# microsoft/Spartan

Hardware: AMD Instinct MI355X
Metric: R1CS constraints/sec in SNARK::prove (synthetic 2^20); bit-exact proof (higher is better)
Workload: dtype u64x4 (F_q Montgomery / F_p 2^255-19 limbs)

## Files before the change

### spartan_amd/csrc/spark.hip

```cpp
#include "internal.hpp"

__global__ void __launch_bounds__(256) k_from_index(const uint32_t* __restrict__ ix, size_t n, Fq* __restrict__ dst) { SP_FG_PRIO();
  for (size_t i = (size_t)blockIdx.x * blockDim.x + threadIdx.x; i < n; i += (size_t)gridDim.x * blockDim.x) st_fq(dst + i, fq_from_u64(ix[i]));
}
__global__ void __launch_bounds__(256) k_gather(const Fq* __restrict__ mem, const uint32_t* __restrict__ addr, size_t n, Fq* __restrict__ dst) { SP_FG_PRIO();
  for (size_t i = (size_t)blockIdx.x * blockDim.x + threadIdx.x; i < n; i += (size_t)gridDim.x * blockDim.x) st_fq(dst + i, ld_fq(mem + addr[i]));
}
__global__ void __launch_bounds__(256) k_hash_layer(const Fq* __restrict__ addr, const Fq* __restrict__ val, const Fq* __restrict__ ts, int ts_inc,
                                                    size_t n, Fq r_hash, Fq r_hash_sqr, Fq r_multiset, Fq* __restrict__ dst) { SP_FG_PRIO();
  for (size_t i = (size_t)blockIdx.x * blockDim.x + threadIdx.x; i < n; i += (size_t)gridDim.x * blockDim.x) {
    Fq a = addr ? ld_fq(addr + i) : fq_from_u64((uint64_t)i);
    Fq t = ts ? ld_fq(ts + i) : fq_zero();
    if (ts_inc) t = fq_add(t, fq_one());
    Fq h = fq_add(fq_add(fq_mul(t, r_hash_sqr), fq_mul(ld_fq(val + i), r_hash)), a);
    st_fq(dst + i, fq_sub(h, r_multiset));
  }
}
template <bool PAIR>
__global__ void __launch_bounds__(256) k_hash_layer_first(const Fq* __restrict__ addr, const Fq* __restrict__ val, const Fq* __restrict__ ts, int ts_inc,
                                                          size_t n, Fq r_hash, Fq r_hash_sqr, Fq r_multiset, Fq* __restrict__ dst_a, Fq* __restrict__ dst_b) { SP_FG_PRIO();
  const size_t half = n / 2;
  for (size_t i = (size_t)blockIdx.x * blockDim.x + threadIdx.x; i < half; i += (size_t)gridDim.x * blockDim.x) {
    Fq h[2];
#pragma unroll
    for (int k = 0; k < 2; k++) {
      const size_t j = i + (size_t)k * half;
      Fq a = addr ? ld_fq(addr + j) : fq_from_u64((uint64_t)j);
      Fq t = ts ? ld_fq(ts + j) : fq_zero();
      if (ts_inc) t = fq_add(t, fq_one());
      h[k] = fq_sub(fq_add(fq_add(fq_mul(t, r_hash_sqr), fq_mul(ld_fq(val + j), r_hash)), a), r_multiset);
      st_fq(dst_a + j, h[k]);
    }
    st_fq(dst_a + n + i, fq_mul(h[0], h[1]));
    if (PAIR) {
      Fq w0 = fq_add(h[0], r_hash_sqr), w1 = fq_add(h[1], r_hash_sqr);
      st_fq(dst_b + i, w0);
      st_fq(dst_b + half + i, w1);
      st_fq(dst_b + n + i, fq_mul(w0, w1));
    }
  }
}
__global__ void __launch_bounds__(256) k_prod_layer(const Fq* __restrict__ in, size_t half, Fq* __restrict__ out) { SP_FG_PRIO();
  for (size_t i = (size_t)blockIdx.x * blockDim.x + threadIdx.x; i < half; i += (size_t)gridDim.x * blockDim.x)
    st_fq(out + i, fq_mul(ld_fq(in + i), ld_fq(in + half + i)));
}

struct Stores16 {
  Fq* p[16];
};
__global__ void __launch_bounds__(256) k_prod_layer_many(Stores16 st, size_t off, size_t half, size_t noff) { SP_FG_PRIO();
  const Fq* in = st.p[blockIdx.y] + off;
  Fq* out = st.p[blockIdx.y] + noff;
  for (size_t i = (size_t)blockIdx.x * blockDim.x + threadIdx.x; i < half; i += (size_t)gridDim.x * blockDim.x)
    st_fq(out + i, fq_mul(ld_fq(in + i), ld_fq(in + half + i)));
}

__global__ void __launch_bounds__(256) k_prod_layer2_many(Stores16 st, size_t off, size_t len) { SP_FG_PRIO();
  const size_t q = len / 4, off1 = off + len, off2 = off1 + len / 2;
  Fq* base = st.p[blockIdx.y];
  for (size_t i = (size_t)blockIdx.x * blockDim.x + threadIdx.x; i < q; i += (size_t)gridDim.x * blockDim.x) {
    const Fq x0 = ld_fq(base + off + i), x1 = ld_fq(base + off + q + i), x2 = ld_fq(base + off + 2 * q + i), x3 = ld_fq(base + off + 3 * q + i);
    const Fq lo = fq_mul(x0, x2), hi = fq_mul(x1, x3);
    st_fq(base + off1 + i, lo);
    st_fq(base + off1 + q + i, hi);
    st_fq(base + off2 + i, fq_mul(lo, hi));
  }
}
__global__ void __launch_bounds__(256) k_prod_layer_tail(Stores16 st, size_t off, size_t len) { SP_FG_PRIO();
  __shared__ Fq cur[1024];
  Fq* base = st.p[blockIdx.x];
  size_t half = len / 2, noff = off + len;
  for (size_t i = threadIdx.x; i < half; i += 256) {
    Fq v = fq_mul(ld_fq(base + off + i), ld_fq(base + off + half + i));
    cur[i] = v;
    st_fq(base + noff + i, v);
  }
  __syncthreads();
  len = half;
  while (len > 2) {
    half = len / 2;
    noff += len;
    Fq v[2];
    int n = 0;
    for (size_t i = threadIdx.x; i < half; i += 256) v[n++] = fq_mul(cur[i], cur[half + i]);
    __syncthreads();
    n = 0;
    for (size_t i = threadIdx.x; i < half; i += 256) { cur[i] = v[n]; st_fq(base + noff + i, v[n]); n++; }
    __syncthreads();
    len = half;
  }
}

struct Triple {
  Fq *a, *b, *c;
  Fq* c_out;
};
struct TripleInline { Triple t[24]; };
__device__ __forceinline__ void cubic_point(const Fq& a0, const Fq& a1, const Fq& b0, const Fq& b1, const Fq& c0, const Fq& c1, Fq (&e)[3]) {
  Fq da = fq_sub(a1, a0), db = fq_sub(b1, b0), dc = fq_sub(c1, c0);
  Fq a2 = fq_add(a1, da), b2 = fq_add(b1, db), c2 = fq_add(c1, dc);
  Fq a3 = fq_add(a2, da), b3 = fq_add(b2, db), c3 = fq_add(c2, dc);
  e[0] = fq_add(e[0], fq_mul(fq_mul(a0, b0), c0));
  e[1] = fq_add(e[1], fq_mul(fq_mul(a2, b2), c2));
  e[2] = fq_add(e[2], fq_mul(fq_mul(a3, b3), c3));
}
__global__ void __launch_bounds__(256) k_cubic_eval_batched(const Triple* __restrict__ T, TripleInline IN, size_t half, Fq* __restrict__ partials) { SP_FG_PRIO();
  __shared__ Fq sm[256];
  Triple t = T ? T[blockIdx.y] : IN.t[blockIdx.y];
  Fq e[3] = {fq_zero(), fq_zero(), fq_zero()};
  for (size_t i = (size_t)blockIdx.x * blockDim.x + threadIdx.x; i < half; i += (size_t)gridDim.x * blockDim.x)
    cubic_point(ld_fq(t.a + i), ld_fq(t.a + half + i), ld_fq(t.b + i), ld_fq(t.b + half + i), ld_fq(t.c + i), ld_fq(t.c + half + i), e);
  block_sum_fq<3>(e, sm);
  if (threadIdx.x == 0) {
    Fq* p = partials + ((size_t)blockIdx.y * gridDim.x + blockIdx.x) * 3;
    st_fq(p, e[0]); st_fq(p + 1, e[1]); st_fq(p + 2, e[2]);
  }
}
__global__ void __launch_bounds__(256) k_cubic_bind_eval_batched(const Triple* __restrict__ T, TripleInline IN, size_t quarter, Fq r, Fq* __restrict__ partials) { SP_FG_PRIO();
  __shared__ Fq sm[256];
  Triple t = T ? T[blockIdx.y] : IN.t[blockIdx.y];
  Fq e[3] = {fq_zero(), fq_zero(), fq_zero()};
  for (size_t i = (size_t)blockIdx.x * blockDim.x + threadIdx.x; i < quarter; i += (size_t)gridDim.x * blockDim.x) {
    Fq lo[3], hi[3];
    Fq* ptr[3] = {t.a, t.b, t.c};
#pragma unroll
    for (int k = 0; k < 3; k++) {
      Fq x0 = ld_fq(ptr[k] + i), x1 = ld_fq(ptr[k] + quarter + i), x2 = ld_fq(ptr[k] + 2 * quarter + i), x3 = ld_fq(ptr[k] + 3 * quarter + i);
      lo[k] = fq_add(x0, fq_mul(r, fq_sub(x2, x0)));
      hi[k] = fq_add(x1, fq_mul(r, fq_sub(x3, x1)));
      if (k < 2) {
        st_fq(ptr[k] + i, lo[k]);
        st_fq(ptr[k] + quarter + i, hi[k]);
      } else if (t.c_out) {
        st_fq(t.c_out + i, lo[k]);
        st_fq(t.c_out + quarter + i, hi[k]);
      }
    }
    cubic_point(lo[0], hi[0], lo[1], hi[1], lo[2], hi[2], e);
  }
  block_sum_fq<3>(e, sm);
  if (threadIdx.x == 0) {
    Fq* p = partials + ((size_t)blockIdx.y * gridDim.x + blockIdx.x) * 3;
    st_fq(p, e[0]); st_fq(p + 1, e[1]); st_fq(p + 2, e[2]);
  }
}
__device__ __forceinline__ void quad_point_eq(const Fq& a0, const Fq& a1, const Fq& b0, const Fq& b1, const Fq& c, Fq (&e)[4]) {
  Fq a2 = fq_add(a1, fq_sub(a1, a0)), b2 = fq_add(b1, fq_sub(b1, b0));
  e[0] = fq_add(e[0], fq_mul(fq_mul(a0, b0), c));
  e[1] = fq_add(e[1], fq_mul(fq_mul(a2, b2), c));
}
__device__ __forceinline__ void cubic_point4(const Fq& a0, const Fq& a1, const Fq& b0, const Fq& b1, const Fq& c0, const Fq& c1, Fq (&e)[4]) {
  Fq da = fq_sub(a1, a0), db = fq_sub(b1, b0), dc = fq_sub(c1, c0);
  Fq a2 = fq_add(a1, da), b2 = fq_add(b1, db), c2 = fq_add(c1, dc);
  Fq a3 = fq_add(a2, da), b3 = fq_add(b2, db), c3 = fq_add(c2, dc);
  e[0] = fq_add(e[0], fq_mul(fq_mul(a0, b0), c0));
  e[1] = fq_add(e[1], fq_mul(fq_mul(a1, b1), c1));
  e[2] = fq_add(e[2], fq_mul(fq_mul(a2, b2), c2));
  e[3] = fq_add(e[3], fq_mul(fq_mul(a3, b3), c3));
}
template <bool GEN>
__global__ void __launch_bounds__(256) k_cubic_eval_batched_eq(TripleInline IN, unsigned inst0, size_t half, Fq* __restrict__ partials) { SP_FG_PRIO();
  __shared__ Fq sm[256];
  const unsigned inst = inst0 + blockIdx.y;
  Triple t = IN.t[inst];
  Fq e[4] = {fq_zero(), fq_zero(), fq_zero(), fq_zero()};
  if (!GEN) {
    for (size_t i = (size_t)blockIdx.x * blockDim.x + threadIdx.x; i < half; i += (size_t)gridDim.x * blockDim.x)
      quad_point_eq(ld_fq(t.a + i), ld_fq(t.a + half + i), ld_fq(t.b + i), ld_fq(t.b + half + i), ld_fq(t.c + i), e);
  } else {
    for (size_t i = (size_t)blockIdx.x * blockDim.x + threadIdx.x; i < half; i += (size_t)gridDim.x * blockDim.x)
      cubic_point4(ld_fq(t.a + i), ld_fq(t.a + half + i), ld_fq(t.b + i), ld_fq(t.b + half + i), ld_fq(t.c + i), ld_fq(t.c + half + i), e);
  }
  if (GEN) block_sum_fq<4>(e, sm);
  else {
    Fq q[2] = {e[0], e[1]};
    block_sum_fq<2>(q, sm);
    e[0] = q[0]; e[1] = q[1];
  }
  if (threadIdx.x == 0) {
    Fq* p = partials + ((size_t)inst * gridDim.x + blockIdx.x) * 4;
    st_fq(p, e[0]); st_fq(p + 1, e[1]); st_fq(p + 2, e[2]); st_fq(p + 3, e[3]);
  }
}
template <bool GEN>
__global__ void __launch_bounds__(256) k_cubic_bind_eval_batched_eq(TripleInline IN, unsigned inst0, size_t quarter, Fq r, Fq* __restrict__ partials) { SP_FG_PRIO();
  __shared__ Fq sm[256];
  const unsigned inst = inst0 + blockIdx.y;
  Triple t = IN.t[inst];
  Fq e[4] = {fq_zero(), fq_zero(), fq_zero(), fq_zero()};
  for (size_t i = (size_t)blockIdx.x * blockDim.x + threadIdx.x; i < quarter; i += (size_t)gridDim.x * blockDim.x) {
    Fq lo[3], hi[3];
    Fq* ptr[3] = {t.a, t.b, t.c};
#pragma unroll
    for (int k = 0; k < 2; k++) {
      Fq x0 = ld_fq(ptr[k] + i), x1 = ld_fq(ptr[k] + quarter + i), x2 = ld_fq(ptr[k] + 2 * quarter + i), x3 = ld_fq(ptr[k] + 3 * quarter + i);
      lo[k] = fq_add(x0, fq_mul(r, fq_sub(x2, x0)));
      hi[k] = fq_add(x1, fq_mul(r, fq_sub(x3, x1)));
      st_fq(ptr[k] + i, lo[k]);
      st_fq(ptr[k] + quarter + i, hi[k]);
    }
    if (!GEN) {
      quad_point_eq(lo[0], hi[0], lo[1], hi[1], ld_fq(t.c + i), e);
    } else {
      Fq x0 = ld_fq(ptr[2] + i), x1 = ld_fq(ptr[2] + quarter + i), x2 = ld_fq(ptr[2] + 2 * quarter + i), x3 = ld_fq(ptr[2] + 3 * quarter + i);
      lo[2] = fq_add(x0, fq_mul(r, fq_sub(x2, x0)));
      hi[2] = fq_add(x1, fq_mul(r, fq_sub(x3, x1)));
      if (t.c_out) {
        st_fq(t.c_out + i, lo[2]);
        st_fq(t.c_out + quarter + i, hi[2]);
      }
      cubic_point4(lo[0], hi[0], lo[1], hi[1], lo[2], hi[2], e);
    }
  }
  if (GEN) block_sum_fq<4>(e, sm);
  else {
    Fq q[2] = {e[0], e[1]};
    block_sum_fq<2>(q, sm);
    e[0] = q[0]; e[1] = q[1];
  }
  if (threadIdx.x == 0) {
    Fq* p = partials + ((size_t)inst * gridDim.x + blockIdx.x) * 4;
    st_fq(p, e[0]); st_fq(p + 1, e[1]); st_fq(p + 2, e[2]); st_fq(p + 3, e[3]);
  }
}
__global__ void __launch_bounds__(256) k_scale_prefix(Fq* __restrict__ t, size_t n, Fq k) { SP_FG_PRIO();
  for (size_t i = (size_t)blockIdx.x * blockDim.x + threadIdx.x; i < n; i += (size_t)gridDim.x * blockDim.x) st_fq(t + i, fq_mul(ld_fq(t + i), k));
}
__global__ void __launch_bounds__(256) k_cubic_bind_eval_tiny(const Triple* __restrict__ T, TripleInline IN, size_t quarter, Fq r, Fq* __restrict__ partials, DoneSig sig) { SP_FG_PRIO();
  __shared__ Fq bound[32][6];
  __shared__ Fq lv[32][3][3];
  __shared__ Fq red[3][32];
  Triple t = T ? T[blockIdx.y] : IN.t[blockIdx.y];
  int li = threadIdx.x >> 3, role = threadIdx.x & 7;
  size_t i = (size_t)blockIdx.x * 32 + li;
  bool live = i < quarter;
  if (role < 6 && live) {
    int k = role >> 1, half = role & 1;
    Fq* ptr = k == 0 ? t.a : (k == 1 ? t.b : t.c);
    Fq x0 = ld_fq(ptr + (size_t)half * quarter + i), x2 = ld_fq(ptr + (size_t)(2 + half) * quarter + i);
    Fq v = fq_add(x0, fq_mul(r, fq_sub(x2, x0)));
    bound[li][role] = v;
    if (k < 2) st_fq(ptr + (size_t)half * quarter + i, v);
    else if (t.c_out) st_fq(t.c_out + (size_t)half * quarter + i, v);
  }
  __syncthreads();
  if (role < 3 && live) {
    const Fq lo = bound[li][2 * role], hi = bound[li][2 * role + 1];
    const Fq d = fq_sub(hi, lo), e2 = fq_add(hi, d), e3 = fq_add(e2, d);
    lv[li][role][0] = lo; lv[li][role][1] = e2; lv[li][role][2] = e3;
  }
  __syncthreads();
  if (role < 3) {
    Fq e = fq_zero();
    if (live) e = fq_mul(fq_mul(lv[li][0][role], lv[li][1][role]), lv[li][2][role]);
    red[role][li] = e;
  }
  __syncthreads();
  for (int s = 16; s > 0; s >>= 1) {
    if (role < 3 && li < s) red[role][li] = fq_add(red[role][li], red[role][li + s]);
    __syncthreads();
  }
  if (threadIdx.x < 3) st_fq(partials + ((size_t)blockIdx.y * gridDim.x + blockIdx.x) * 3 + threadIdx.x, red[threadIdx.x][0]);
  signal_done(sig);
}
__global__ void __launch_bounds__(256) k_cubic_eval_tiny(const Triple* __restrict__ T, TripleInline IN, size_t half, Fq* __restrict__ partials, DoneSig sig) { SP_FG_PRIO();
  __shared__ Fq red[3][64];
  Triple t = T ? T[blockIdx.y] : IN.t[blockIdx.y];
  int li = threadIdx.x >> 2, role = threadIdx.x & 3;
  size_t i = (size_t)blockIdx.x * 64 + li;
  Fq e = fq_zero();
  if (role < 3 && i < half) {
    Fq pt[3];
    const Fq* ptr[3] = {t.a, t.b, t.c};
#pragma unroll
    for (int k = 0; k < 3; k++) {
      Fq x0 = ld_fq(ptr[k] + i), x1 = ld_fq(ptr[k] + half + i);
      Fq x2 = fq_sub(fq_dbl(x1), x0), x3 = fq_sub(fq_add(x2, x1), x0);
#pragma unroll
      for (int w = 0; w < 4; w++) pt[k].l[w] = role == 0 ? x0.l[w] : (role == 1 ? x2.l[w] : x3.l[w]);
    }
    e = fq_mul(fq_mul(pt[0], pt[1]), pt[2]);
  }
  if (role < 3) red[role][li] = e;
  __syncthreads();
  for (int s = 32; s > 0; s >>= 1) {
    if (role < 3 && li < s) red[role][li] = fq_add(red[role][li], red[role][li + s]);
    __syncthreads();
  }
  if (threadIdx.x < 3) st_fq(partials + ((size_t)blockIdx.y * gridDim.x + blockIdx.x) * 3 + threadIdx.x, red[threadIdx.x][0]);
  signal_done(sig);
}

struct Triple2 {
  Fq *a, *b, *c;
  Fq* c_out;
};
__device__ __forceinline__ Fq line_at(const Fq& u, const Fq& v, int t) {
  Fq x2 = fq_sub(fq_dbl(v), u), x3 = fq_sub(fq_add(x2, v), u), r;
#pragma unroll
  for (int w = 0; w < 4; w++) r.l[w] = t == 0 ? u.l[w] : (t == 1 ? x2.l[w] : x3.l[w]);
  return r;
}
struct Bind2Inline {
  Triple2 t[24];
  Fq w[24];
};
__global__ void __launch_bounds__(256) k_cubic_bind2_eval(const Triple2* __restrict__ T, Bind2Inline IN, const Fq* __restrict__ weights, size_t len, int nbind, Fq r0, Fq r1,
                                                          Fq* __restrict__ partials, Fq* __restrict__ dump, DoneSig sig) { SP_FG_PRIO();
  __shared__ Fq first[8][12][2];
  __shared__ Fq bnd[8][12];
  __shared__ Fq red[18][8];
  __shared__ Fq lv[8][3][6][3];
  DoneSig kt = sig; if (blockIdx.x != 0 || blockIdx.y != 0) kt.kt = nullptr;
  SP_KT(kt, 0);
  const Triple2 t = T ? T[blockIdx.y] : IN.t[blockIdx.y];
  const Fq wv = !weights ? fq_zero() : (T ? ld_fq(weights + blockIdx.y) : IN.w[blockIdx.y]);
  const int grp = threadIdx.x >> 5, lane = threadIdx.x & 31;
  const size_t n2 = len >> nbind;
  const size_t np = n2 < 4 ? n2 : 4, ng = n2 / np;
  const size_t g = (size_t)blockIdx.x * 8 + grp;
  const bool live = g < ng;
  Fq* const ptr[3] = {t.a, t.b, t.c};
  if (nbind) {
    if (nbind == 2) {
      if (live && lane < 24) {
        const int k = lane >> 3, p = (lane >> 1) & 3, h = lane & 1;
        if ((size_t)p < np) {
          const size_t y = g + (size_t)p * ng + (size_t)h * (len / 4);
          Fq lo = ld_fq(ptr[k] + y), hi = ld_fq(ptr[k] + y + len / 2);
          SP_KT(kt, 1);
          first[grp][k * 4 + p][h] = fq_add(lo, fq_mul(r0, fq_sub(hi, lo)));
        }
      }
      SP_KT(kt, 2);
      __syncthreads();
    }
    if (live && lane < 12) {
      const int k = lane >> 2, p = lane & 3;
      if ((size_t)p < np) {
        Fq lo, hi;
        if (nbind == 2) { lo = first[grp][lane][0]; hi = first[grp][lane][1]; }
        else { lo = ld_fq(ptr[k] + g + (size_t)p * ng); hi = ld_fq(ptr[k] + g + (size_t)p * ng + len / 2); }
        Fq v = fq_add(lo, fq_mul(nbind == 2 ? r1 : r0, fq_sub(hi, lo)));
        const size_t z = g + (size_t)p * ng;
        if (k < 2) st_fq(ptr[k] + z, v);
        else if (t.c_out) st_fq(t.c_out + z, v);
        if (dump) st_fq(dump + ((size_t)blockIdx.y * 3 + k) * 8 + z, v);
        bnd[grp][k * 4 + (np == 2 && p == 1 ? 2 : p)] = v;
      }
    }
  } else if (live && lane < 12) {
    const int k = lane >> 2, p = lane & 3;
    if ((size_t)p < np) {
      const Fq v = ld_fq(ptr[k] + g + (size_t)p * ng);
      if (dump) st_fq(dump + ((size_t)blockIdx.y * 3 + k) * 8 + g + (size_t)p * ng, v);
      bnd[grp][k * 4 + (np == 2 && p == 1 ? 2 : p)] = v;
    }
  }
  SP_KT(kt, 3);
  __syncthreads();
  if (live && lane < 12 && np >= 2) {
    const int k = lane >> 2, line = lane & 3;
    if (line == 0 || np == 4) {
      const int iu = line == 0 ? 0 : (line == 1 ? 1 : (line == 2 ? 0 : 2)), iv = line == 0 ? 2 : (line == 1 ? 3 : (line == 2 ? 1 : 3));
// ... 176 lines not shown
    size_t half = len / 2, noff = off + len;
    ProfScope ps(c, PF_SPARK, 48.0 * (double)len);
    hipLaunchKernelGGL(k_prod_layer, dim3((unsigned)grid_for(half)), dim3(256), 0, c->stream, (const Fq*)(store->d + off), half, store->d + noff);
    off = noff;
    len = half;
  }
  return hipGetLastError() == hipSuccess ? SP_OK : SP_EHIP;
}

int32_t sp_product_tree_many(sp_ctx* c, sp_table* const* stores, size_t count, size_t n) { return sp_product_tree_many_from(c, stores, count, n, 0); }
int32_t sp_product_tree_many_from(sp_ctx* c, sp_table* const* stores, size_t count, size_t n, size_t layers_done) {
  if (!c || !stores || count == 0 || !is_pow2(n) || n < 2 || layers_done > 1 || (layers_done == 1 && n < 4)) return SP_EINVAL;
  for (size_t k = 0; k < count; k++)
    if (!stores[k] || stores[k]->cap < 2 * n) return SP_EINVAL;
  HIPCHK(hipSetDevice(c->dev));
  for (size_t k0 = 0; k0 < count; k0 += 16) {
    size_t nk = count - k0 < 16 ? count - k0 : 16;
    Stores16 st;
    for (size_t k = 0; k < 16; k++) st.p[k] = k < nk ? stores[k0 + k]->d : nullptr;
    size_t off = 0, len = n;
    if (layers_done == 1) { off = n; len = n / 2; }
    while (len > 2) {
      size_t half = len / 2, noff = off + len;
      ProfScope ps(c, PF_SPARK, 48.0 * (double)len * (double)nk);
      if (len <= 2048) {
        hipLaunchKernelGGL(k_prod_layer_tail, dim3((unsigned)nk), dim3(256), 0, c->stream, st, off, len);
        break;
      }
      const bool two_layers = c->opt.v[OPT_SPARK_PROD_LAYER2] != 0;
      const size_t l2max = (size_t)1 << (c->opt.v[OPT_SPARK_PROD_LAYER2_MAX_LOG2] < 13 ? 13 : c->opt.v[OPT_SPARK_PROD_LAYER2_MAX_LOG2]);
      if (two_layers && len <= l2max && len >= 8192) {
        hipLaunchKernelGGL(k_prod_layer2_many, dim3((unsigned)grid_for(len / 4, 1024), (unsigned)nk), dim3(256), 0, c->stream, st, off, len);
        off = off + len + len / 2;
        len = len / 4;
        continue;
      }
      hipLaunchKernelGGL(k_prod_layer_many, dim3((unsigned)grid_for(half, 1024), (unsigned)nk), dim3(256), 0, c->stream, st, off, half, noff);
      off = noff;
      len = half;
    }
  }
  return hipGetLastError() == hipSuccess ? SP_OK : SP_EHIP;
}

static int32_t batched_setup(sp_ctx* c, sp_table* const* A, sp_table* const* B, sp_table* const* C, size_t ninst, size_t* len_out, bool bind_c, TripleInline* IN,
                             const Triple** Tdev) {
  if (!c || !A || !B || !C || ninst == 0 || ninst > 64) return SP_EINVAL;
  size_t len = A[0] ? A[0]->len : 0;
  std::vector<Triple> T(ninst);
  for (size_t k = 0; k < ninst; k++) {
    if (!A[k] || !B[k] || !C[k] || A[k]->len != len || B[k]->len != len || C[k]->len != len) return SP_EINVAL;
    T[k] = Triple{A[k]->d, B[k]->d, C[k]->d, nullptr};
  }
  if (len < 2 || !is_pow2(len)) return SP_EINVAL;
  if (bind_c) {
    for (size_t k = 0; k < ninst; k++) {
      bool first = true;
      for (size_t m = 0; m < k; m++) first = first && C[m] != C[k];
      if (first) {
        SPCHK(table_ensure_alt(C[k], len / 2));
        T[k].c_out = C[k]->alt;
      }
    }
  }
  const bool inline_args = c->opt.v[OPT_SUMCHECK_INLINE_ARGS] != 0;
  if (inline_args && ninst <= 24) {
    memcpy(IN->t, T.data(), sizeof(Triple) * ninst);
    *Tdev = nullptr;
  } else {
    stage_small(c, 0, T.data(), sizeof(Triple) * ninst);
    *Tdev = (const Triple*)c->hmap;
  }
  *len_out = len;
  return SP_OK;
}
static bool host_sums(size_t nblk, size_t ninst) { return nblk == 1 || 96 * nblk * ninst <= HOST_SUM_BYTES; }
static int32_t batched_finish(sp_ctx* c, Fq* partials, size_t nblk, size_t ninst, uint64_t* out, const DoneSig& sig) {
  if (partials != (Fq*)hres(c)) {
    {
      ProfScope ps(c, PF_REDUCE, 96.0 * (double)(nblk * ninst));
      hipLaunchKernelGGL(k_reduce_partials_batched, dim3((unsigned)ninst), dim3(256), 0, c->stream, (const Fq*)partials, nblk, 3, (Fq*)hres(c), sig);
    }
    SPCHK(sig_wait(c, sig));
    memcpy(out, hres(c), 96 * ninst);
    return hipGetLastError() == hipSuccess ? SP_OK : SP_EHIP;
  }
  SPCHK(sig_wait(c, sig));
  if (hipGetLastError() != hipSuccess) return SP_EHIP;
  const Fq* p = (const Fq*)hres(c);
  Fq* o = (Fq*)out;
  for (size_t i = 0; i < ninst; i++)
    for (int k = 0; k < 3; k++) {
      Fq acc = p[(i * nblk) * 3 + k];
      for (size_t b = 1; b < nblk; b++) acc = fq_add(acc, p[(i * nblk + b) * 3 + k]);
      o[3 * i + k] = acc;
    }
  return SP_OK;
}
int32_t sp_sumcheck_eval_batched(sp_ctx* c, sp_table* const* A, sp_table* const* B, sp_table* const* C, size_t ninst, uint64_t* out) {
  if (!out) return SP_EINVAL;
  size_t len;
  HIPCHK(hipSetDevice(c ? c->dev : 0));
  TripleInline IN;
  const Triple* Tdev = nullptr;
  SPCHK(batched_setup(c, A, B, C, ninst, &len, false, &IN, &Tdev));
  size_t half = len / 2;
  bool tiny = half <= 8192;
  size_t nblk = tiny ? (half + 63) / 64 : grid_for(half, 256);
  SPCHK(ensure(&c->scratch, &c->scratch_cap, 32 * 3 * (nblk + 1) * ninst));
  bool on_host = host_sums(nblk, ninst) && tiny;
  Fq* partials = on_host ? (Fq*)hres(c) : (Fq*)c->scratch;
  DoneSig sig = sig_make(c, on_host ? nblk * ninst : ninst);
  {
    ProfScope ps(c, PF_SC_EVAL, 96.0 * (double)len * (double)ninst, nullptr, 6.0 * (double)half * (double)ninst);
    if (tiny) hipLaunchKernelGGL(k_cubic_eval_tiny, dim3((unsigned)nblk, (unsigned)ninst), dim3(256), 0, c->stream, Tdev, IN, half, partials, on_host ? sig : sig_none());
    else hipLaunchKernelGGL(k_cubic_eval_batched, dim3((unsigned)nblk, (unsigned)ninst), dim3(256), 0, c->stream, Tdev, IN, half, partials);
  }
  return batched_finish(c, partials, nblk, ninst, out, sig);
}
int32_t sp_sumcheck_bind_eval_batched(sp_ctx* c, sp_table* const* A, sp_table* const* B, sp_table* const* C, size_t ninst, const uint64_t r[4],
                                      uint64_t* out) {
  if (!out || !r) return SP_EINVAL;
  size_t len;
  HIPCHK(hipSetDevice(c ? c->dev : 0));
  if (!c) return SP_EINVAL;
  for (size_t k = 0; k < ninst && C; k++)
    if (C[k] && C[k]->len < 4) return SP_EINVAL;
  TripleInline IN;
  const Triple* Tdev = nullptr;
  SPCHK(batched_setup(c, A, B, C, ninst, &len, true, &IN, &Tdev));
  if (len < 4) return SP_EINVAL;
  size_t quarter = len / 4;
  bool tiny = quarter <= 8192;
  size_t nblk = tiny ? (quarter + 31) / 32 : grid_for(quarter, 256);
  SPCHK(ensure(&c->scratch, &c->scratch_cap, 32 * 3 * (nblk + 1) * ninst));
  bool on_host = host_sums(nblk, ninst) && tiny;
  Fq* partials = on_host ? (Fq*)hres(c) : (Fq*)c->scratch;
  DoneSig sig = sig_make(c, on_host ? nblk * ninst : ninst);
  {
    ProfScope ps(c, PF_SC_BIND_EVAL, (96.0 + 32.0) * (double)len * (double)ninst, nullptr, 12.0 * (double)quarter * (double)ninst);
    if (tiny)
      hipLaunchKernelGGL(k_cubic_bind_eval_tiny, dim3((unsigned)nblk, (unsigned)ninst), dim3(256), 0, c->stream, Tdev, IN, quarter,
                         limbs(r), partials, on_host ? sig : sig_none());
    else
      hipLaunchKernelGGL(k_cubic_bind_eval_batched, dim3((unsigned)nblk, (unsigned)ninst), dim3(256), 0, c->stream, Tdev, IN, quarter,
                         limbs(r), partials);
  }
  for (size_t k = 0; k < ninst; k++) { A[k]->len = len / 2; B[k]->len = len / 2; }
  for (size_t k = 0; k < ninst; k++)
    if (C[k]->len == len) table_swap_to_alt(C[k], len / 2);
  return batched_finish(c, partials, nblk, ninst, out, sig);
}

static int32_t batched_finish4(sp_ctx* c, Fq* partials, size_t nblk, size_t ninst, uint64_t* out, const DoneSig& sig) {
  {
    ProfScope ps(c, PF_REDUCE, 128.0 * (double)(nblk * ninst));
    hipLaunchKernelGGL(k_reduce_partials_batched, dim3((unsigned)ninst), dim3(256), 0, c->stream, (const Fq*)partials, nblk, 4, (Fq*)hres(c), sig);
  }
  SPCHK(sig_wait(c, sig));
  memcpy(out, hres(c), 128 * ninst);
  return hipGetLastError() == hipSuccess ? SP_OK : SP_EHIP;
}
static int32_t eq_form_check(sp_table* const* C, size_t ninst, size_t neq, size_t len) {
  if (neq == 0 || neq > ninst || ninst > 24 || 128 * ninst > HOST_SUM_BYTES) return SP_EINVAL;
  for (size_t k = 0; k < neq; k++)
    if (C[k] != C[0]) return SP_EINVAL;
  if (!C[0] || C[0]->len < len) return SP_EINVAL;
  for (size_t k = neq; k < ninst; k++)
    if (!C[k] || C[k]->len != len || C[k] == C[0]) return SP_EINVAL;
  return SP_OK;
}
static int32_t eq_form_setup(sp_ctx* c, sp_table* const* A, sp_table* const* B, sp_table* const* C, size_t ninst, size_t neq, bool bind_c, size_t* len_out,
                             TripleInline* IN) {
  if (!c || !A || !B || !C || ninst == 0) return SP_EINVAL;
  const size_t len = A[0] ? A[0]->len : 0;
  if (len < 65536 || !is_pow2(len)) return SP_EINVAL;
  SPCHK(eq_form_check(C, ninst, neq, len));
  for (size_t k = 0; k < ninst; k++) {
    if (!A[k] || !B[k] || A[k]->len != len || B[k]->len != len) return SP_EINVAL;
    IN->t[k] = Triple{A[k]->d, B[k]->d, C[k]->d, nullptr};
    if (bind_c && k >= neq) {
      bool first = true;
      for (size_t m = neq; m < k; m++) first = first && C[m] != C[k];
      if (first) {
        SPCHK(table_ensure_alt(C[k], len / 2));
        IN->t[k].c_out = C[k]->alt;
      }
    }
  }
  *len_out = len;
  return SP_OK;
}
int32_t sp_sumcheck_eval_batched_eq(sp_ctx* c, sp_table* const* A, sp_table* const* B, sp_table* const* C, size_t ninst, size_t neq, uint64_t* out) {
  if (!c || !out) return SP_EINVAL;
  HIPCHK(hipSetDevice(c->dev));
  size_t len;
  TripleInline IN;
  SPCHK(eq_form_setup(c, A, B, C, ninst, neq, false, &len, &IN));
  const size_t half = len / 2, nblk = grid_for(half, 256);
  SPCHK(ensure(&c->scratch, &c->scratch_cap, 32 * 4 * (nblk + 1) * ninst));
  Fq* partials = (Fq*)c->scratch;
  DoneSig sig = sig_make(c, ninst);
  {
    ProfScope ps(c, PF_SC_EVAL, 32.0 * (double)len * (2.5 * (double)neq + 3.0 * (double)(ninst - neq)), nullptr,
                 (double)half * (4.0 * (double)neq + 8.0 * (double)(ninst - neq)));
    hipLaunchKernelGGL(k_cubic_eval_batched_eq<false>, dim3((unsigned)nblk, (unsigned)neq), dim3(256), 0, c->stream, IN, 0u, half, partials);
    if (ninst > neq)
      hipLaunchKernelGGL(k_cubic_eval_batched_eq<true>, dim3((unsigned)nblk, (unsigned)(ninst - neq)), dim3(256), 0, c->stream, IN, (unsigned)neq, half, partials);
  }
  return batched_finish4(c, partials, nblk, ninst, out, sig);
}
int32_t sp_sumcheck_bind_eval_batched_eq(sp_ctx* c, sp_table* const* A, sp_table* const* B, sp_table* const* C, size_t ninst, size_t neq, const uint64_t r[4],
                                         uint64_t* out) {
  if (!c || !out || !r) return SP_EINVAL;
  HIPCHK(hipSetDevice(c->dev));
  size_t len;
  TripleInline IN;
  SPCHK(eq_form_setup(c, A, B, C, ninst, neq, true, &len, &IN));
  const size_t quarter = len / 4, nblk = grid_for(quarter, 256);
  SPCHK(ensure(&c->scratch, &c->scratch_cap, 32 * 4 * (nblk + 1) * ninst));
  Fq* partials = (Fq*)c->scratch;
  DoneSig sig = sig_make(c, ninst);
  {
    ProfScope ps(c, PF_SC_BIND_EVAL, 32.0 * (double)len * (3.25 * (double)neq + 4.0 * (double)(ninst - neq)), nullptr,
                 (double)quarter * (8.0 * (double)neq + 14.0 * (double)(ninst - neq)));
    hipLaunchKernelGGL(k_cubic_bind_eval_batched_eq<false>, dim3((unsigned)nblk, (unsigned)neq), dim3(256), 0, c->stream, IN, 0u, quarter, limbs(r), partials);
    if (ninst > neq)
      hipLaunchKernelGGL(k_cubic_bind_eval_batched_eq<true>, dim3((unsigned)nblk, (unsigned)(ninst - neq)), dim3(256), 0, c->stream, IN, (unsigned)neq, quarter,
                         limbs(r), partials);
  }
  for (size_t k = 0; k < ninst; k++) { A[k]->len = len / 2; B[k]->len = len / 2; }
  for (size_t k = neq; k < ninst; k++)
    if (C[k]->len == len) table_swap_to_alt(C[k], len / 2);
  return batched_finish4(c, partials, nblk, ninst, out, sig);
}
int32_t sp_table_scale_prefix(sp_ctx* c, sp_table* t, size_t n, const uint64_t k[4]) {
  if (!c || !t || !k || n == 0 || n > t->len) return SP_EINVAL;
  HIPCHK(hipSetDevice(c->dev));
  {
    ProfScope ps(c, PF_MISC, 64.0 * (double)n);
    hipLaunchKernelGGL(k_scale_prefix, dim3((unsigned)grid_for(n)), dim3(256), 0, c->stream, t->d, n, limbs(k));
  }
  t->len = n;
  return hipGetLastError() == hipSuccess ? SP_OK : SP_EHIP;
}

__global__ void __launch_bounds__(256) k_reduce_partials18(const Fq* __restrict__ partials, size_t nblk, Fq* __restrict__ out, DoneSig sig) { SP_FG_PRIO();
  __shared__ Fq sm[8][18];
  const int k = threadIdx.x & 31, sl = threadIdx.x >> 5;
  const Fq* p = partials + (size_t)blockIdx.x * nblk * 18;
  if (k < 18) {
    Fq acc = fq_zero();
    for (size_t b = sl; b < nblk; b += 8) acc = fq_add(acc, ld_fq(p + b * 18 + k));
    sm[sl][k] = acc;
  }
  __syncthreads();
  if (threadIdx.x < 18) {
    Fq acc = sm[0][threadIdx.x];
#pragma unroll
    for (int j = 1; j < 8; j++) acc = fq_add(acc, sm[j][threadIdx.x]);
    st_fq(out + (size_t)blockIdx.x * 18 + threadIdx.x, acc);
  }
  signal_done(sig);
}
constexpr size_t TAIL_OFF = 12288, TAIL_MAX_INST = 21;
struct Bind2Shape {
  size_t n2, nblk;
  bool host, tail;
};
static Bind2Shape bind2_shape(size_t len, int nbind, size_t ninst, bool want_tables) {
  Bind2Shape s;
  s.n2 = len >> nbind;
  const size_t np = s.n2 < 4 ? s.n2 : 4, ng = s.n2 / np;
  s.nblk = (ng + 7) / 8;
  s.host = 32 * 18 * s.nblk * ninst <= HOST_SUM_BYTES;
  s.tail = want_tables && s.n2 >= 2 && s.n2 <= 8 && ninst <= TAIL_MAX_INST && s.host && s.nblk == 1;
  return s;
}
static void bind2_enqueue(sp_ctx* c, const Bind2Inline& IN, bool inl, const Fq* dweights, size_t len, int nbind, const Fq& r0, const Fq& r1, size_t ninst,
                          const Bind2Shape& sh, const DoneSig& sig) {
  const size_t ng = sh.n2 / (sh.n2 < 4 ? sh.n2 : 4);
  Fq* partials = sh.host ? (Fq*)hres(c) : (Fq*)c->scratch;
  Fq* dump = sh.tail ? (Fq*)(hres(c) + TAIL_OFF) : nullptr;
  {
    ProfScope ps(c, nbind ? PF_SC_BIND_EVAL : PF_SC_EVAL, 96.0 * (double)len * (double)ninst, nullptr, (nbind ? 36.0 + 36.0 : 36.0) * (double)ng * (double)ninst);
    hipLaunchKernelGGL(k_cubic_bind2_eval, dim3((unsigned)sh.nblk, (unsigned)ninst), dim3(256), 0, c->stream, inl ? (const Triple2*)nullptr : (const Triple2*)c->hmap, IN, dweights, len,
                       nbind, r0, r1, partials, dump, sh.host ? sig : sig_none());
  }
  if (!sh.host) {
    ProfScope ps(c, PF_REDUCE, 32.0 * 18 * (double)(sh.nblk * ninst));
    hipLaunchKernelGGL(k_reduce_partials18, dim3((unsigned)ninst), dim3(256), 0, c->stream, (const Fq*)partials, sh.nblk, (Fq*)hres(c), sig);
  }
}
static int32_t bind2_launch(sp_ctx* c, sp_table* const* A, sp_table* const* B, sp_table* const* C, size_t ninst, int nbind, const uint64_t* r0, const uint64_t* r1,
                            const uint64_t* weights, uint64_t* out_evals, uint64_t* out_coeffs, uint64_t* out_heads, uint64_t* out_tables = nullptr) {
  if (!c || !A || !B || !C || ninst == 0 || ninst > 64) return SP_EINVAL;
  HIPCHK(hipSetDevice(c->dev));
  size_t len = A[0] ? A[0]->len : 0;
  if (len < ((size_t)1 << nbind) || len < 2 || !is_pow2(len)) return SP_EINVAL;
  const int do_bind = nbind;
  const size_t n2 = len >> nbind;
  if ((n2 >= 2 && !out_evals) || (n2 >= 4 && !out_coeffs) || (n2 == 1 && !out_heads)) return SP_EINVAL;
  for (size_t k = 0; k < ninst; k++)
    if (!A[k] || !B[k] || !C[k] || A[k]->len != len || B[k]->len != len || C[k]->len != len) return SP_EINVAL;
  std::vector<Triple2> T(ninst);
  std::vector<sp_table*> distinctC;
  for (size_t k = 0; k < ninst; k++) {
    T[k] = Triple2{A[k]->d, B[k]->d, C[k]->d, nullptr};
    bool first = true;
    for (size_t m = 0; m < k; m++) first = first && C[m] != C[k];
    if (first) {
      distinctC.push_back(C[k]);
      if (do_bind) {
        SPCHK(table_ensure_alt(C[k], n2));
        T[k].c_out = C[k]->alt;
      }
    }
  }
  const bool inline_args = c->opt.v[OPT_SUMCHECK_INLINE_ARGS] != 0;
  const bool inl = inline_args && ninst <= 24;
  Bind2Inline IN;
  const Fq* dweights = nullptr;
  if (inl) {
    memcpy(IN.t, T.data(), sizeof(Triple2) * ninst);
    if (weights) { memcpy(IN.w, weights, 32 * ninst); dweights = (const Fq*)c->hmap; }
  } else {
    stage_small(c, 0, T.data(), sizeof(Triple2) * ninst);
    dweights = weights ? (const Fq*)stage_small(c, sizeof(Triple2) * 64, weights, 32 * ninst) : nullptr;
  }
  const Bind2Shape sh = bind2_shape(len, nbind, ninst, out_tables != nullptr);
  const Fq z = fq_zero();
  SPCHK(ensure(&c->scratch, &c->scratch_cap, 32 * 18 * (sh.nblk + 1) * ninst));
  const DoneSig sig = sig_make(c, sh.host ? sh.nblk * ninst : ninst);
  bind2_enqueue(c, IN, inl, dweights, len, nbind, r0 ? limbs(r0) : z, r1 ? limbs(r1) : z, ninst, sh, sig);
  if (do_bind) {
    for (size_t k = 0; k < ninst; k++) { A[k]->len = n2; B[k]->len = n2; }
    for (sp_table* t : distinctC) table_swap_to_alt(t, n2);
  }
  SPCHK(sig_wait(c, sig));
  std::vector<Fq> sums(18 * ninst);
  if (!sh.host) {
    memcpy(sums.data(), hres(c), 32 * 18 * ninst);
  } else {
    const Fq* p = (const Fq*)hres(c);
    for (size_t i = 0; i < ninst; i++)
      for (int k = 0; k < 18; k++) {
        Fq acc = p[(i * sh.nblk) * 18 + k];
        for (size_t b = 1; b < sh.nblk; b++) acc = fq_add(acc, p[(i * sh.nblk + b) * 18 + k]);
        sums[18 * i + k] = acc;
      }
  }
  if (hipGetLastError() != hipSuccess) return SP_EHIP;
  if (out_tables) {
    if (sh.tail) {
      const Fq* d = (const Fq*)(hres(c) + TAIL_OFF);
      for (size_t i = 0; i < ninst; i++)
        for (int k = 0; k < 3; k++) memcpy(out_tables + 4 * ((i * 3 + k) * n2), d + (i * 3 + k) * 8, 32 * n2);
    } else {
      out_tables[0] = ~0ULL;
    }
  }
  if (weights) {
    Fq tot[15];
    for (int k = 0; k < 15; k++) {
      Fq acc = sums[k];
      for (size_t i = 1; i < ninst; i++) acc = fq_add(acc, sums[18 * i + k]);
      tot[k] = acc;
    }
    if (n2 >= 2) memcpy(out_evals, tot, 96);
    if (n2 >= 4) memcpy(out_coeffs, tot + 3, 384);
  }
  for (size_t i = 0; i < ninst; i++) {
// ... 92 lines not shown
```

Baseline: 47.21 million.

## Prefetch next grid-stride loads in eq sumcheck kernels and size grids per CU

The batched eq-form sumcheck eval and bind-eval kernels now software-pipeline their grid-stride loops, loading the next iteration's operands into registers before computing on the current ones. The grid for these kernels is now sized from the CU count (about two workgroups per CU spread across instances, with a minimum number of trips per thread) instead of one thread per element. The aim is to hide memory latency and cut the cost of per-block partial reductions. The prefetch raises register pressure on these u64x4 field kernels, which could lower occupancy or cause spills.

```diff
diff --git a/spartan_amd/csrc/spark.hip b/spartan_amd/csrc/spark.hip
--- a/spartan_amd/csrc/spark.hip
+++ b/spartan_amd/csrc/spark.hip
@@ -158,18 +158,41 @@
   e[2] = fq_add(e[2], fq_mul(fq_mul(a2, b2), c2));
   e[3] = fq_add(e[3], fq_mul(fq_mul(a3, b3), c3));
 }
+struct FqPair { Fq lo, hi; };
+struct FqQuad { Fq x0, x1, x2, x3; };
+__device__ __forceinline__ FqPair ld_pair(const Fq* p, size_t half, size_t i) { return FqPair{ld_fq(p + i), ld_fq(p + half + i)}; }
+__device__ __forceinline__ FqQuad ld_quad(const Fq* p, size_t quarter, size_t i) {
+  return FqQuad{ld_fq(p + i), ld_fq(p + quarter + i), ld_fq(p + 2 * quarter + i), ld_fq(p + 3 * quarter + i)};
+}
+__device__ __forceinline__ FqPair bind_quad(const FqQuad& q, const Fq& r) {
+  return FqPair{fq_add(q.x0, fq_mul(r, fq_sub(q.x2, q.x0))), fq_add(q.x1, fq_mul(r, fq_sub(q.x3, q.x1)))};
+}
 template <bool GEN>
 __global__ void __launch_bounds__(256) k_cubic_eval_batched_eq(TripleInline IN, unsigned inst0, size_t half, Fq* __restrict__ partials) { SP_FG_PRIO();
   __shared__ Fq sm[256];
   const unsigned inst = inst0 + blockIdx.y;
   Triple t = IN.t[inst];
   Fq e[4] = {fq_zero(), fq_zero(), fq_zero(), fq_zero()};
-  if (!GEN) {
-    for (size_t i = (size_t)blockIdx.x * blockDim.x + threadIdx.x; i < half; i += (size_t)gridDim.x * blockDim.x)
-      quad_point_eq(ld_fq(t.a + i), ld_fq(t.a + half + i), ld_fq(t.b + i), ld_fq(t.b + half + i), ld_fq(t.c + i), e);
-  } else {
-    for (size_t i = (size_t)blockIdx.x * blockDim.x + threadIdx.x; i < half; i += (size_t)gridDim.x * blockDim.x)
-      cubic_point4(ld_fq(t.a + i), ld_fq(t.a + half + i), ld_fq(t.b + i), ld_fq(t.b + half + i), ld_fq(t.c + i), ld_fq(t.c + half + i), e);
+  const size_t stride = (size_t)gridDim.x * blockDim.x;
+  size_t i = (size_t)blockIdx.x * blockDim.x + threadIdx.x;
+  FqPair na = {fq_zero(), fq_zero()}, nb = na, nc = na;
+  if (i < half) {
+    na = ld_pair(t.a, half, i);
+    nb = ld_pair(t.b, half, i);
+    nc.lo = ld_fq(t.c + i);
+    if (GEN) nc.hi = ld_fq(t.c + half + i);
+  }
+  for (; i < half; i += stride) {
+    const FqPair a = na, b = nb, c = nc;
+    const size_t j = i + stride;
+    if (j < half) {
+      na = ld_pair(t.a, half, j);
+      nb = ld_pair(t.b, half, j);
+      nc.lo = ld_fq(t.c + j);
+      if (GEN) nc.hi = ld_fq(t.c + half + j);
+    }
+    if (!GEN) quad_point_eq(a.lo, a.hi, b.lo, b.hi, c.lo, e);
+    else cubic_point4(a.lo, a.hi, b.lo, b.hi, c.lo, c.hi, e);
   }
   if (GEN) block_sum_fq<4>(e, sm);
   else {
@@ -188,28 +211,48 @@
   const unsigned inst = inst0 + blockIdx.y;
   Triple t = IN.t[inst];
   Fq e[4] = {fq_zero(), fq_zero(), fq_zero(), fq_zero()};
-  for (size_t i = (size_t)blockIdx.x * blockDim.x + threadIdx.x; i < quarter; i += (size_t)gridDim.x * blockDim.x) {
-    Fq lo[3], hi[3];
-    Fq* ptr[3] = {t.a, t.b, t.c};
-#pragma unroll
-    for (int k = 0; k < 2; k++) {
-      Fq x0 = ld_fq(ptr[k] + i), x1 = ld_fq(ptr[k] + quarter + i), x2 = ld_fq(ptr[k] + 2 * quarter + i), x3 = ld_fq(ptr[k] + 3 * quarter + i);
-      lo[k] = fq_add(x0, fq_mul(r, fq_sub(x2, x0)));
-      hi[k] = fq_add(x1, fq_mul(r, fq_sub(x3, x1)));
-      st_fq(ptr[k] + i, lo[k]);
-      st_fq(ptr[k] + quarter + i, hi[k]);
-    }
+  const size_t stride = (size_t)gridDim.x * blockDim.x;
+  size_t i = (size_t)blockIdx.x * blockDim.x + threadIdx.x;
+  const FqQuad z4 = {fq_zero(), fq_zero(), fq_zero(), fq_zero()};
+  FqQuad na = z4, nb = z4;
+  Fq nc = fq_zero();
+  if (i < quarter) {
+    na = ld_quad(t.a, quarter, i);
     if (!GEN) {
-      quad_point_eq(lo[0], hi[0], lo[1], hi[1], ld_fq(t.c + i), e);
+      nb = ld_quad(t.b, quarter, i);
+      nc = ld_fq(t.c + i);
+    }
+  }
+  for (; i < quarter; i += stride) {
+    FqQuad qb = nb, qc = z4;
+    if (GEN) {
+      qb = ld_quad(t.b, quarter, i);
+      qc = ld_quad(t.c, quarter, i);
+    }
+    const FqQuad qa = na;
+    const Fq c = nc;
+    const size_t j = i + stride;
+    if (j < quarter) {
+      na = ld_quad(t.a, quarter, j);
+      if (!GEN) {
+        nb = ld_quad(t.b, quarter, j);
+        nc = ld_fq(t.c + j);
+      }
+    }
+    const FqPair a = bind_quad(qa, r), b = bind_quad(qb, r);
+    st_fq(t.a + i, a.lo);
+    st_fq(t.a + quarter + i, a.hi);
+    st_fq(t.b + i, b.lo);
+    st_fq(t.b + quarter + i, b.hi);
+    if (!GEN) {
+      quad_point_eq(a.lo, a.hi, b.lo, b.hi, c, e);
     } else {
-      Fq x0 = ld_fq(ptr[2] + i), x1 = ld_fq(ptr[2] + quarter + i), x2 = ld_fq(ptr[2] + 2 * quarter + i), x3 = ld_fq(ptr[2] + 3 * quarter + i);
-      lo[2] = fq_add(x0, fq_mul(r, fq_sub(x2, x0)));
-      hi[2] = fq_add(x1, fq_mul(r, fq_sub(x3, x1)));
+      const FqPair cc = bind_quad(qc, r);
       if (t.c_out) {
-        st_fq(t.c_out + i, lo[2]);
-        st_fq(t.c_out + quarter + i, hi[2]);
+        st_fq(t.c_out + i, cc.lo);
+        st_fq(t.c_out + quarter + i, cc.hi);
       }
-      cubic_point4(lo[0], hi[0], lo[1], hi[1], lo[2], hi[2], e);
+      cubic_point4(a.lo, a.hi, b.lo, b.hi, cc.lo, cc.hi, e);
     }
   }
   if (GEN) block_sum_fq<4>(e, sm);
@@ -692,6 +735,19 @@
   return batched_finish(c, partials, nblk, ninst, out, sig);
 }
 
+constexpr size_t ROUND_WG_PER_CU = 2, ROUND_MIN_TRIPS = 4;
+static size_t round_blocks(const sp_ctx* c, size_t idx, size_t ninst) {
+  const size_t cus = (size_t)c->n_cus;
+  size_t bx = cus * ROUND_WG_PER_CU / ninst;
+  if (bx > idx / (256 * ROUND_MIN_TRIPS)) bx = idx / (256 * ROUND_MIN_TRIPS);
+  if (bx < (cus + ninst - 1) / ninst) bx = (cus + ninst - 1) / ninst;
+  if (bx > (idx + 255) / 256) bx = (idx + 255) / 256;
+  return bx ? bx : 1;
+}
+static size_t round_blocks_eq(const sp_ctx* c, size_t idx, size_t ninst, size_t neq) {
+  const size_t ngen = ninst - neq;
+  return round_blocks(c, idx, ngen && ngen < neq ? ngen : neq);
+}
 static int32_t batched_finish4(sp_ctx* c, Fq* partials, size_t nblk, size_t ninst, uint64_t* out, const DoneSig& sig) {
   {
     ProfScope ps(c, PF_REDUCE, 128.0 * (double)(nblk * ninst));
@@ -737,7 +793,7 @@
   size_t len;
   TripleInline IN;
   SPCHK(eq_form_setup(c, A, B, C, ninst, neq, false, &len, &IN));
-  const size_t half = len / 2, nblk = grid_for(half, 256);
+  const size_t half = len / 2, nblk = round_blocks_eq(c, half, ninst, neq);
   SPCHK(ensure(&c->scratch, &c->scratch_cap, 32 * 4 * (nblk + 1) * ninst));
   Fq* partials = (Fq*)c->scratch;
   DoneSig sig = sig_make(c, ninst);
@@ -757,7 +813,7 @@
   size_t len;
   TripleInline IN;
   SPCHK(eq_form_setup(c, A, B, C, ninst, neq, true, &len, &IN));
-  const size_t quarter = len / 4, nblk = grid_for(quarter, 256);
+  const size_t quarter = len / 4, nblk = round_blocks_eq(c, quarter, ninst, neq);
   SPCHK(ensure(&c->scratch, &c->scratch_cap, 32 * 4 * (nblk + 1) * ninst));
   Fq* partials = (Fq*)c->scratch;
   DoneSig sig = sig_make(c, ninst);
```

Result: no change. 47.20 million (-0.0%).
